# minaskar/pocomc

Hardware: AMD Instinct MI355X
Metric: preconditioned MCMC steps/sec (1e4 particles, 32-D) (higher is better)
Workload: dtype f32 flow (MFMA) + f64 step

## Files before the change

include/pocomc_amd.h:

```cpp
#ifndef POCOMC_AMD_H
#define POCOMC_AMD_H

#include <stdint.h>

#ifdef __cplusplus
extern "C" {
#endif

#define PMC_ABI_VERSION 9

const char* pmc_last_error(void);
int pmc_abi_version(void);
const char* pmc_build_id(void);


typedef struct pmc_maf {
    const float* packed;
    const int32_t* meta;
    int32_t D, H, T;
    int32_t Hp, Dp;
    int32_t nT, nXT, nOT;
    int64_t pk_per_transform;
    int32_t tri_ok;
    int32_t n_out;
    const uint16_t* lane16;
    int32_t lane16_fmt;
    int32_t reserved;
} pmc_maf_t;

#define PMC_MAF_VARIANT_LEFT_LOOKING 1
#define PMC_MAF_VARIANT_LANE_FOUR 2

#define PMC_INVERSE_AUTO 0
#define PMC_INVERSE_TRIANGULAR 1
#define PMC_INVERSE_NAIVE 2
#define PMC_INVERSE_TRIANGULAR_SOLO 6
#define PMC_INVERSE_TRIANGULAR_LANE 8
#define PMC_INVERSE_TRIANGULAR_LANE16 9
#define PMC_INVERSE_TRIANGULAR_DUO 7

int pmc_maf_pack(const float* flat, const int32_t* pack_idx, float* packed, int64_t n_packed, void* stream);

int pmc_maf_forward(const pmc_maf_t* m, const float* x, float* z, float* ladj, float* log_prob,
                    int64_t n, void* stream);

int pmc_maf_pack_bf16(const float* flat, const int32_t* pack_idx, uint16_t* image, int64_t n, void* stream);
// ... 280 lines not shown

#define PMC_ADAPT_TPCN 1
#define PMC_ADAPT_PRWM 2
#define PMC_ADAPT_RWM 3
#define PMC_ADAPT_MU 8

int pmc_rng_fill(const pmc_rng_t* rng, double gamma_shape, double* normal, double* gamma, double* uniform,
                 int64_t n, int32_t D, void* stream);
int pmc_event_synchronize(void* ev);

int pmc_propose_inverse(int kind, const float* cur32, const double* mu, const double* inv_cov, const double* chol,
                        double nu, double sigma, double cn_a, const pmc_rng_t* rng, double* prop64, double* quad,
                        double* quad_prop, const pmc_maf_t* maf, float* u_out, float* ladj, int64_t n, void* stream);

int pmc_step_pre(const pmc_step_t* s, const pmc_rng_t* rng, double nu, double sigma, double cn_a, void* stream);
int pmc_step_post(const pmc_step_t* s, const pmc_rng_t* rng, double beta, double nu, int want_mask,
                  int copy_sums, void* stream);
int pmc_step_lik_rows(const pmc_step_t* s, void* stream);
int pmc_step_prior_rows(const pmc_step_t* s, const void* logp, int logp_is_f32, void* stream);
int pmc_adapt_update(const double* const* parts, int32_t n_parts, int32_t D, double* total_out, double* h_sums,
                     double* adapt_state, int32_t adapt_mode, double c_sigma, double c_mu, double cap, double n_total,
                     const pmc_done_t* done, void* stream);
int pmc_stream_synchronize(void* stream);

void* pmc_comm_create(int32_t rank, int32_t world, int32_t width);
void* pmc_comm_create_host(int32_t rank, int32_t world, int32_t width);
int pmc_comm_kind(void* comm);
int pmc_comm_unlink(void* comm);
int pmc_comm_handle(void* comm, void* out64);
int pmc_comm_connect(void* comm, const void* handles);
// ... 82 lines not shown
```

pocomc_amd/_lib.py:

```python
from __future__ import annotations

import ctypes as C
import os

_HERE = os.path.dirname(os.path.abspath(__file__))
LIB_PATH = os.environ.get("PMC_LIBRARY") or os.path.join(_HERE, "libpocomc_amd.so")

c_p = C.c_void_p


class pmc_maf_t(C.Structure):
    _fields_ = [("packed", c_p), ("meta", c_p),
                ("D", C.c_int32), ("H", C.c_int32), ("T", C.c_int32),
                ("Hp", C.c_int32), ("Dp", C.c_int32),
                ("nT", C.c_int32), ("nXT", C.c_int32), ("nOT", C.c_int32),
                ("pk_per_transform", C.c_int64),
                ("tri_ok", C.c_int32), ("n_out", C.c_int32),
                ("lane16", c_p), ("lane16_fmt", C.c_int32), ("reserved", C.c_int32)]


class pmc_maf_train_t(C.Structure):
    _fields_ = [("packedT", c_p), ("gmap", c_p), ("pkT_per_transform", C.c_int64),
                ("gmap_per_transform", C.c_int64),
                ("jobs", c_p), ("n_jobs", C.c_int32), ("max_sets", C.c_int32), ("n_sq_partial", C.c_int32),
# ... 110 lines not shown
    "pmc_scaler_forward": (C.c_int, [P(pmc_scaler_t), c_p, c_p, i64, c_p]),
    "pmc_prior_logpdf": (C.c_int, [P(pmc_prior_t), c_p, c_p, c_p, i64, c_p]),
    "pmc_scaler_inverse_prior": (C.c_int, [P(pmc_scaler_t), P(pmc_prior_t), c_p, c_p, c_p, c_p, c_p, c_p, c_p, c_p,
                                           c_p, c_p, P(pmc_done_t), i64, c_p]),
    "pmc_wait_flag": (C.c_int, [c_p, i64, f64]),
    "pmc_propose": (C.c_int, [C.c_int, c_p, c_p, c_p, c_p, c_p, f64, f64, f64, P(pmc_rng_t),
                              c_p, c_p, c_p, c_p, i64, i32, c_p]),
    "pmc_accept_workspace_bytes": (i64, [i64, i32]),
    "pmc_accept": (C.c_int, [C.c_int, C.c_int, P(pmc_state_t), P(pmc_proposal_t), f64, f64,
                             P(pmc_rng_t), c_p, c_p, c_p, c_p, i64, i32, c_p]),
    "pmc_accept_armed": (C.c_int, [C.c_int, C.c_int, P(pmc_state_t), P(pmc_proposal_t), f64, f64,
                                   P(pmc_rng_t), c_p, c_p, c_p, c_p, P(pmc_done_t), c_p, i64, i32, c_p]),
    "pmc_propose_inverse": (C.c_int, [C.c_int, c_p, c_p, c_p, c_p, f64, f64, f64, P(pmc_rng_t), c_p, c_p, c_p,
                                      P(pmc_maf_t), c_p, c_p, i64, c_p]),
    "pmc_step_pre": (C.c_int, [P(pmc_step_t), P(pmc_rng_t), f64, f64, f64, c_p]),
    "pmc_step_post": (C.c_int, [P(pmc_step_t), P(pmc_rng_t), f64, f64, C.c_int, C.c_int, c_p]),
    "pmc_step_lik_rows": (C.c_int, [P(pmc_step_t), c_p]),
    "pmc_step_prior_rows": (C.c_int, [P(pmc_step_t), c_p, C.c_int, c_p]),
    "pmc_stream_synchronize": (C.c_int, [c_p]),
    "pmc_pipeline_create": (C.c_void_p, [C.POINTER(C.c_void_p), i32, C.c_uint64, C.POINTER(C.c_uint64), c_p, f64, c_p]),
    "pmc_pipeline_set_comm": (C.c_int, [c_p, c_p]),
    "pmc_comm_create": (C.c_void_p, [i32, i32, i32]),
    "pmc_comm_create_host": (C.c_void_p, [i32, i32, i32]),
    "pmc_comm_kind": (C.c_int, [c_p]),
    "pmc_comm_unlink": (C.c_int, [c_p]),
    "pmc_comm_handle": (C.c_int, [c_p, c_p]),
    "pmc_comm_connect": (C.c_int, [c_p, c_p]),
    "pmc_comm_destroy": (None, [c_p]),
    "pmc_comm_adapt_update": (C.c_int, [c_p, C.POINTER(C.c_void_p), i32, i32, c_p, c_p, c_p, i32, f64, f64, f64, f64, P(pmc_done_t), f64,
                                        c_p]),
# ... 120 lines not shown
```

pocomc_amd/csrc/maf_inverse_tri4.hip:

```cpp

#include <stdlib.h>
#include "maf_chain_rot.h"

#define DG_WORDS(m) ((m)->nT * 4 + 8)
#define TRI5_TT_WORDS(m) (((m)->nT + 2) * 16)
#define TRI5_YT_WORDS(m) ((m)->T * (((m)->nT + 2) * 4 + 1))
#define TRI5_TABLE_WORDS(m) (((TRI5_TT_WORDS(m) + (m)->Dp + 2 * (m)->T + 3) & ~3) + (m)->Dp * 16 + ((TRI5_YT_WORDS(m) + 3) & ~3))
#define TRI5_LDS_FLOATS(m, maxo) (2 * (m)->Dp * 16 + 2 * (m)->Hp * 16 + 2 * 256 + 2 * (3 + (maxo)) * 256 + TRI5_TABLE_WORDS(m))
#include "propose_body.h"

#define PX4 2
#define PK4 8


template <int TT>
__device__ __forceinline__ void burst_tile_open(f32x4& a1, f32x4& a2, f32x4& c1, f32x4& c2, const float4 (&pf1)[PK4],
                                                const float4 (&pf2)[PK4], const float* H0, const float* H1, int lane) {
    if constexpr (TT > 0) {
        float4 b1[TT], b2[TT];
#pragma unroll
        for (int i = 0; i < TT; ++i) {
            b1[i] = *reinterpret_cast<const float4*>(H0 + (i << 8) + (lane << 2));
            b2[i] = *reinterpret_cast<const float4*>(H1 + (i << 8) + (lane << 2));
        }
// ... 514 lines not shown
        else if constexpr (K == 11) F.w0o[3] = make_float4(0.f, 0.f, 0.f, 0.f);
        else F.w0N[K - 12] = bload4(rs, U + 1 < nT ? ((K - 12) << 6) + vo_q : OOB_VOFF, base + oCW0 + Un * 1024);
    };
    auto take_table = [&](ChainFrags<MAXO>& F, const int tt, const int U) {
        const int4 ty = *reinterpret_cast<const int4*>(YT + (tt * (nT + 2) + U) * 4);
        F.yo[0] = ty.x; F.yo[1] = ty.y; F.yo[2] = ty.z; F.yo[3] = ty.w;
        const int4 tg = *reinterpret_cast<const int4*>(DGT + 16 * U);
        const int4 txy = *reinterpret_cast<const int4*>(DGT + 16 * U + 4);
        const int4 tso = *reinterpret_cast<const int4*>(DGT + 16 * U + 8);
        F.g[0] = tg.x & 0xffff; F.g[1] = tg.y; F.g[2] = tg.z; F.g[3] = tg.w;
        F.pat = tg.x >> 16;
        F.xy[0] = txy.x; F.xy[1] = txy.y; F.xy[2] = txy.z; F.xy[3] = txy.w;
        F.so[0] = tso.x; F.so[1] = tso.y; F.so[2] = tso.z; F.so[3] = tso.w;
    };

    ChainFrags<MAXO> fA, fB;
    if (wv < TRI5_NC) {
        fill_table();
        WAVE_LDS_FENCE();
        {
            auto woff = [](const int r) { return 4 * (((r >> 4) << 8) + ((r & 3) << 6) + ((r >> 2) & 3)); };
            auto src_rank = [&](const int tt, const int g) {
                if (g >= D) return 0;
                return tt == T - 1 ? g : rank_of_feat[(tt + 1) * D + feat_of_rank[tt * D + g]];
            };
            for (int e = lane; e < T * (nT + 2) * 4; e += 64) {
                const int tt = e / ((nT + 2) * 4), rem = e - tt * (nT + 2) * 4;
                YT[e] = woff(src_rank(tt, DGT[16 * (rem >> 2) + (rem & 3)] & 0xffff));
            }
            for (int tt = lane; tt < T; tt += 64) Y0T[tt] = woff(src_rank(tt, 0));
        }
        WAVE_LDS_FENCE();
        {
            const int4 w0 = *reinterpret_cast<const int4*>(DGT + 12), w1 = *reinterpret_cast<const int4*>(DGT + 16 + 12);
            take_table(fA, T - 1, 0);
            static_for<16>([&](auto k_) { request(fA, k_, T - 1, 0, w0, w1); });
        }
        if constexpr (FM > 0) {
            for (int e = lane; e < (Dp - D) * 16; e += 64) Y[lidx(D + (e >> 4), e & 15)] = 0.0f;
            const double sg = pa.adapt ? pa.adapt[0] : pa.sigma, ca = pa.adapt ? pa.adapt[1] : pa.cn_a;
            propose_body<FM>(pa.kind, pa.cur32, nullptr, pa.adapt ? pa.adapt + 2 : pa.mu, pa.inv_cov, pa.chol, pa.nu, sg,
                             ca, pa.rng, pa.prop64, nullptr, pa.quad, pa.quad_prop, n, D, Y, rank_of_feat + (T - 1) * D,
                             set);
        } else {
            load_rows(Y, in, row0, n, D, Dp, feat_of_rank + (T - 1) * D, lane);
        }
    } else {
        float4* z4 = reinterpret_cast<float4*>(H0);
        const int n4 = (2 * Hp * 16 + 2 * 256 + 2 * TRI5_STAGE_FLOATS(MAXO)) >> 2;
        for (int e = lane; e < n4; e += 64) z4[e] = make_float4(0.f, 0.f, 0.f, 0.f);
    }
    if (pa.prof && lane == 0 && blockIdx.x < 64)
        pa.prof[(size_t)T * nT * 8 + blockIdx.x * 2 + wv] = (long long)__builtin_amdgcn_s_getreg((31 << 11) | 4);
    for (int r = threadIdx.x; r < D; r += 64 * (TRI5_NC + 1)) PRM[r] = feat_of_rank[r];
    for (int tt = threadIdx.x; tt < T; tt += 64 * (TRI5_NC + 1)) {
        const float* b3 = m.packed + (size_t)tt * m.pk_per_transform + (oB3 >> 2);
        B3T[2 * tt] = b3[0];
        B3T[2 * tt + 1] = b3[1];
    }
    for (int e = threadIdx.x; e < (Dp * 16) >> 2; e += 64 * (TRI5_NC + 1)) {
        reinterpret_cast<float4*>(XA)[e] = make_float4(0.f, 0.f, 0.f, 0.f);
        reinterpret_cast<float4*>(XB)[e] = make_float4(0.f, 0.f, 0.f, 0.f);
    }
    float ladj = 0.0f;
    int xsel = 0;
    __syncthreads();

#define BURST_FETCH(TB, TT, P1, P2, XF, OF, Bz0, Bz1, Bz2)                                                        \
            {    \
                 \
                const int TT_ = (TT) < nT ? (TT) : nT - 1;                                                        \
                const int so1_ = (TB) + oF1 + TT_ * nT * 1024, so2_ = (TB) + oF2 + TT_ * nT * 1024;               \
                _Pragma("unroll") for (int i_ = 0; i_ < PK4; ++i_) {                                              \
// ... 305 lines not shown
```

pocomc_amd/csrc/scaler_body.h:

```cpp
#ifndef PMC_SCALER_BODY_H
#define PMC_SCALER_BODY_H

#include <hip/hip_runtime.h>
#include <math.h>
#include <stdint.h>
#include "../../include/pocomc_amd.h"

#pragma clang fp contract(off)

#define LOG_SQRT_2PI 0.91893853320467267
#define SQRT2 1.4142135623730951

__device__ __forceinline__ double np_pairwise_leaf(const double* a, int n) {
    if (n < 8) {
        double res = 0.0;
        for (int i = 0; i < n; ++i) res += a[i];
        return res;
    }
    double r0 = a[0], r1 = a[1], r2 = a[2], r3 = a[3], r4 = a[4], r5 = a[5], r6 = a[6], r7 = a[7];
    int i;
    for (i = 8; i < n - (n % 8); i += 8) {
        r0 += a[i + 0]; r1 += a[i + 1]; r2 += a[i + 2]; r3 += a[i + 3];
        r4 += a[i + 4]; r5 += a[i + 5]; r6 += a[i + 6]; r7 += a[i + 7];
    }
// ... 124 lines not shown
    }
    e.u_out[g] = u;
    e.x_out[g] = x;
    if (direct_cm) { if (e.x_colmajor) e.x_colmajor[(size_t)j * n + row0 + r] = x; }
    else Xt[j * 17 + r] = x;
    Jt[r * D + j] = J;
    if (e.have_prior) Pt[r * D + j] = prior_term(e.pr, j, x);
    if (!isfinite(x)) rowfin[r] = 0;
}

__device__ __forceinline__ void scaler_epilogue_rows(const ScalerEpi& e, const double* Jt, const double* Pt, const double* Xt,
                                                     int* rowfin, int64_t row0, int64_t n, int D, int tid, int nthr,
                                                     bool cm_done) {
    const pmc_scaler_t& s = e.s;
    const int rows = (int)min((int64_t)16, n - row0);
    if (tid < rows) {
        double l = np_pairwise_sum(Jt + (size_t)tid * D, D);
        if (s.scale) l = s.sum_log_sigma + l;
        e.ldj_out[row0 + tid] = l;
        const int fin = (rowfin[tid] && isfinite(l)) ? 1 : 0;
        e.finite_out[row0 + tid] = fin;
        if (e.finite_copy) e.finite_copy[row0 + tid] = fin;
        bool clean = fin != 0;
        if (e.have_prior) {
            double lp = -INFINITY;
            if (fin) {
                lp = 0.0;
                for (int j = 0; j < D; ++j) lp += Pt[tid * D + j];
            }
            e.logp_out[row0 + tid] = lp;
            if (e.logp_copy) e.logp_copy[row0 + tid] = lp;
            clean = clean && isfinite(lp);
        }
        if (e.bad_count && !clean) atomicAdd(e.bad_count, 1u);
        if (e.fill_x) rowfin[tid] = clean ? 1 : 0;
    }
    if (e.fill_x) __syncthreads();
    if (e.stamps && tid == 0) e.stamps[blockIdx.x * 8 + 2] = wall_clock64();
    if (e.stamps && tid == 0) e.stamps[blockIdx.x * 8 + 3] = wall_clock64();
    if (e.x_colmajor && !cm_done) {
        for (int el = tid; el < rows * D; el += nthr) {
            const int j = el / rows, r = el - j * rows;
            e.x_colmajor[(size_t)j * n + row0 + r] = (e.fill_x && !rowfin[r]) ? e.fill_x[(row0 + r) * D + j] : Xt[j * 17 + r];
        }
    }
    if (e.stamps && tid == 0) e.stamps[blockIdx.x * 8 + 4] = wall_clock64();
    if (e.done_flag) {
        __builtin_amdgcn_fence(__ATOMIC_RELEASE, "agent");
        __syncthreads();
        if (e.stamps && tid == 0) e.stamps[blockIdx.x * 8 + 5] = wall_clock64();
        if (tid == 0) {
            const unsigned t = __hip_atomic_fetch_add(e.done_ticket, 1u, __ATOMIC_ACQ_REL, __HIP_MEMORY_SCOPE_AGENT);
            if (t == gridDim.x - 1) {
                *e.done_ticket = 0u;
                if (e.bad_count && e.bad_flag) {
                    const unsigned bad = __hip_atomic_exchange(e.bad_count, 0u, __ATOMIC_ACQ_REL, __HIP_MEMORY_SCOPE_AGENT);
                    *e.bad_flag = (long long)bad;
                }
// ... 4 lines not shown
    }
}

template <class LIDX>
__device__ __forceinline__ void scaler_epilogue(const ScalerEpi& e, const float* X, const int* __restrict__ rof,
                                                double* scr, int64_t row0, int64_t n, int D, int tid, int nthr,
                                                LIDX lidx_of) {
    double* Jt = scr;
    double* Pt = Jt + 16 * D;
    double* Xt = Pt + 16 * D;
    int* rowfin = reinterpret_cast<int*>(Xt + D * 17);
    const int rows = (int)min((int64_t)16, n - row0);
    if (tid < 16) rowfin[tid] = 1;
    if (e.stamps && tid == 0) e.stamps[blockIdx.x * 8 + 0] = wall_clock64();
    __syncthreads();
    for (int el = tid; el < rows * D; el += nthr) {
        const int r = el / D, j = el - r * D;
        scaler_epilogue_element(e, Jt, Pt, Xt, rowfin, X[lidx_of(rof[j], r)], r, j, row0, n, D, false);
    }
    __syncthreads();
    if (e.stamps && tid == 0) e.stamps[blockIdx.x * 8 + 1] = wall_clock64();
    scaler_epilogue_rows(e, Jt, Pt, Xt, rowfin, row0, n, D, tid, nthr, false);
}

static inline size_t scaler_progressive_lds_bytes(int D) { return (size_t)(2 * 16 * D) * sizeof(double) + 16 * sizeof(int); }

#endif
```

pocomc_amd/csrc/step.hip:

```cpp

#include <hip/hip_runtime.h>
#include <time.h>
#include "pmc_internal.h"
#include "scaler_body.h"

#ifdef PMC_DEBUG_HOOKS
static long long* g_epilogue_stamps = nullptr;
static int64_t g_epilogue_stamps_n = 0;
#endif

extern "C" int pmc_step_pre(const pmc_step_t* s, const pmc_rng_t* rng, double nu, double sigma, double cn_a,
                            void* stream) {
    if (!s || !rng) return pmc_fail("pmc_step_pre: null argument");
    hipStream_t st = (hipStream_t)stream;
    const int64_t n = s->n;
    const int32_t D = s->D;
    const bool tpcn = (s->kind == PMC_KIND_TPCN);
    pmc_rng_t rr = *rng;
    const bool prefill = s->rng_ready && s->rng_normal[0] && s->rng_normal[1] && s->rng_uniform[0] &&
                         s->rng_uniform[1] && (!tpcn || (s->rng_gamma[0] && s->rng_gamma[1])) && !rng->normal &&
                         !rng->gamma && !rng->uniform;
    const int rb = (int)(rng->step & 1);
    const double gshape = tpcn ? 0.5 * ((double)D + nu) : 0.0;
    if (prefill) {
        if (*s->rng_ready != (int64_t)rng->step) {
            int rcf = pmc_rng_fill(rng, gshape, s->rng_normal[rb], s->rng_gamma[rb], s->rng_uniform[rb], n, D, stream);
            if (rcf) return rcf;
        }
        rr.normal = s->rng_normal[rb];
        rr.gamma = tpcn ? s->rng_gamma[rb] : nullptr;
        rng = &rr;
    }
    auto finish = [&]() -> int {
        if (s->ev_pre_done) (void)hipEventRecord((hipEvent_t)s->ev_pre_done, st);
        if (prefill) {
            pmc_rng_t nx = *rng;
            nx.normal = nullptr; nx.gamma = nullptr; nx.uniform = nullptr;
            nx.step = rng->step + 1;
            int rcf = pmc_rng_fill(&nx, gshape, s->rng_normal[rb ^ 1], s->rng_gamma[rb ^ 1], s->rng_uniform[rb ^ 1], n, D,
                                   stream);
            if (rcf) return rcf;
            *s->rng_ready = (int64_t)nx.step;
        }
        return 0;
    };
    const bool direct = s->host_direct && !s->p_xT;
    const double* mu = s->mu;
    const double* adapt = (s->adapt_state && s->adapt_mode) ? s->adapt_state : nullptr;
    if (!adapt && tpcn && s->h_mu) {
        if (direct) mu = s->h_mu;
        else if (hipMemcpyAsync((void*)s->mu, s->h_mu, (size_t)D * sizeof(double), hipMemcpyHostToDevice, st) != hipSuccess)
            return pmc_fail("pmc_step_pre: H2D mu");
    }
    int rc;
    bool fused = false;
    int scaled = 0;
    const pmc_prior_t* pr = s->prior;
    double* lp = pr ? s->p_logp : nullptr;
// ... 64 lines not shown
                                         lp, fin2, lp2, done, n, stream, &sx);
    }
    if (rc) return rc;
    if (direct || devlik) return finish();
    if (pr) {
        if (hipMemcpyAsync(s->h_logp_out, s->p_logp, (size_t)n * sizeof(double), hipMemcpyDeviceToHost, st) != hipSuccess)
            return pmc_fail("pmc_step_pre: D2H logp");
    }
    const double* xsrc = s->p_xT ? s->p_xT : s->p_x;
    if (hipMemcpyAsync(s->h_x, xsrc, (size_t)n * D * sizeof(double), hipMemcpyDeviceToHost, st) != hipSuccess ||
        hipMemcpyAsync(s->h_fin, s->p_fin, (size_t)n * sizeof(int32_t), hipMemcpyDeviceToHost, st) != hipSuccess)
        return pmc_fail("pmc_step_pre: D2H");
    return finish();
}

__global__ __launch_bounds__(256) void lik_rows_kernel(const double* __restrict__ x_prop, const double* __restrict__ x_cur,
                                                       const int32_t* __restrict__ fin, const double* __restrict__ logp,
                                                       double* __restrict__ lik_x, unsigned* __restrict__ bad_count,
                                                       int64_t n, int D) {
    const int64_t r = (int64_t)blockIdx.x * 256 + threadIdx.x;
    if (r >= n) return;
    const bool reach = fin[r] && isfinite(logp[r]);
    const double* src = (reach ? x_prop : x_cur) + r * D;
    for (int j = 0; j < D; ++j) lik_x[(size_t)j * n + r] = src[j];
    if (!reach) atomicAdd(bad_count, 1u);
}

extern "C" int pmc_step_lik_rows(const pmc_step_t* s, void* stream) {
    if (!s || !s->lik_x || !s->clean_count || !s->p_x || !s->cur.x || !s->p_fin || !s->p_logp || !s->h_logp || s->D < 1)
        return pmc_fail("pmc_step_lik_rows: needs lik_x, clean_count, p_x, cur.x, p_fin, p_logp and h_logp");
// ... 219 lines not shown

extern "C" void pmc_pipeline_destroy(void* pp) { delete (pmc_pipeline*)pp; }

extern "C" int pmc_pipeline_set_comm(void* pp, void* comm) {
    pmc_pipeline* p = (pmc_pipeline*)pp;
    if (!p) return pmc_fail("pmc_pipeline_set_comm: null pipeline");
    p->comm = comm;
    return 0;
}

static int pipeline_enqueue_pre(pmc_pipeline* p, int64_t step, double nu) {
    for (int k = 0; k < p->n_lanes; ++k) {
        pmc_step_t s = *p->lanes[k];
        s.adapt_mode = 1;
        p->rng[k].step = (uint64_t)step;
        const int rc = pmc_step_pre(&s, &p->rng[k], nu, 0.0, 0.0, p->stream);
        if (rc) return rc;
        if (p->prefetcher)
            (void)pmc_prefetcher_submit(p->prefetcher, s.h_done, step + 1, s.h_x, (int64_t)s.n * s.D * 8, p->timeout > 0 ? p->timeout : 1.0);
    }
    return 0;
}

extern "C" int pmc_pipeline_start(void* pp, double nu, int64_t first_step) {
    pmc_pipeline* p = (pmc_pipeline*)pp;
    if (!p) return pmc_fail("pmc_pipeline_start: null pipeline");
    p->step = first_step;
    return pipeline_enqueue_pre(p, first_step, nu);
}

extern "C" int pmc_pipeline_next(void* pp, int32_t lane_done, double beta, double nu, int32_t adapt_mode, double c_sigma,
                                 double c_mu, double cap, double n_total, int32_t more) {
    pmc_pipeline* p = (pmc_pipeline*)pp;
    if (!p || lane_done < -1 || lane_done >= p->n_lanes) return pmc_fail("pmc_pipeline_next: bad argument");
// ... 56 lines not shown
```

pocomc_amd/flow.py:

```python
from __future__ import annotations

import ctypes as C
import warnings

import numpy as np
import torch

from . import _lib
from .maf_spec import MAFSpec, SPEC_BY_NAME, NSF_BY_NAME, spec_by_name


def torch_double_to_float(x: torch.Tensor, warn: bool = True) -> torch.Tensor:
    if x.dtype == torch.float64 and warn:
        warnings.warn("Float64 data is currently unsupported, casting to Float32. "
                      "Output will also have type Float32.")
        return x.float()
    elif x.dtype == torch.float32:
        return x
    raise ValueError(f"Unsupported datatype for input data: {x.dtype}")


LANE16_BOUND = 1e-2
LANE16_LADJ_BOUND = 1e-1
LANE16_LADJ_Q99_BOUND = 5e-2
# ... 16 lines not shown
        self.spec = spec
        self.lib = _lib.load()
        self.device = torch.device(device) if device is not None else _lib.require_gpu()
        if self.device.type != "cuda":
            raise _lib.PocomcAmdError("Flow lives on the GPU; there is no CPU fallback")
        if seed is None:
            seed = int(torch.randint(0, 2 ** 31 - 1, (1,)).item())
        self.params = torch.from_numpy(spec.init_params(seed)).to(self.device)
        self._pack_idx = torch.from_numpy(spec.pack_index()).to(self.device)
        self._meta = torch.from_numpy(spec.device_meta()).to(self.device)
        self._packed = torch.zeros(spec.pk_size, dtype=torch.float32, device=self.device)
        self._desc = _lib.pmc_maf_t(
            packed=self._packed.data_ptr(), meta=self._meta.data_ptr(),
            D=spec.n_dim, H=spec.hidden, T=spec.n_transforms, Hp=spec.Hp, Dp=spec.Dp,
            nT=spec.nT, nXT=spec.nXT, nOT=spec.nOT, pk_per_transform=spec.pk_per_transform,
            tri_ok=int(spec.tri_ok), n_out=spec.n_out)
        self.inverse_algo = 0
        if precision not in ("f32", "bf16"):
            raise ValueError("precision must be 'f32' or 'bf16'")
        if precision == "bf16" and spec.univariate != "affine":
            raise NotImplementedError("the bf16 kernels are built for the affine flows")
        self.precision = precision
        if train_engine not in (None, "f32", "bf16"):
            raise ValueError("train_engine must be None, 'f32' or 'bf16'")
        self.train_engine = train_engine
        if inverse_precision is None:
            inverse_precision = "f32"
        if inverse_precision not in ("f32", "bf16", "f16"):
            raise ValueError("inverse_precision must be 'f32', 'bf16' or 'f16'")
        if inverse_precision != "f32" and spec.univariate != "affine":
            raise NotImplementedError("the 16-bit helper products are built for the affine flows")
# ... 188 lines not shown
```

pocomc_amd/maf_spec.py:

```python
from __future__ import annotations

import math
from dataclasses import dataclass, field

import numpy as np

LOG_SLOPE = math.log(1e-3)


def next_power_of_2(n: int) -> int:
    return 1 if n == 0 else 2 ** (int(n) - 1).bit_length()


def default_hidden(n_dim: int) -> int:
    return max(next_power_of_2(3 * n_dim), 32)


def _ceil_to(x: int, m: int) -> int:
    return (x + m - 1) // m * m


@dataclass
class MAFSpec:

# ... 275 lines not shown
                    b3i[r, :NO] = base_c + off3 + NO * feat + np.arange(NO)
                put("f3i", f3i); put("b3i", b3i)
        return idx.astype(np.int32)

    def tile_groups(self):
        out = []
        for T in range(self.nT):
            dq = self.quad_deg[4 * T:4 * T + 4]
            g = []
            for d in dq:
                if d < self.n_dim and (not g or g[-1] != d):
                    g.append(int(d))
            out.append(g)
        return out

    def device_meta(self) -> np.ndarray:
        D, T = self.n_dim, self.n_transforms
        live = int(np.sum((self.quad_deg.reshape(-1, 4) < D).any(axis=1)))
        hdr = np.array([D, self.hidden, T, self.Hp, self.Dp, self.nT,
                        self.pk_per_transform, live], dtype=np.int32)
        f_o_r = np.concatenate([np.argsort(o) for o in self.orders]).astype(np.int32)
        r_o_f = np.concatenate(self.orders).astype(np.int32)
        return np.concatenate([hdr, f_o_r, r_o_f, self.quad_meta]).astype(np.int32)

    def bf16_layout(self):
        nX2, nK2 = -(-self.Dp // 32), -(-self.Hp // 32)
        sz = {"g0": self.nT * nX2 * 512, "g1": self.nT * nK2 * 512, "g2": self.nT * nK2 * 512, "g3": self.nOT * nK2 * 512}
        off, o = {}, 0
        for k, v in sz.items():
            off[k] = o
            o += v
        return dict(nX2=nX2, nK2=nK2, sz=sz, off=off, per_transform=o)

    def pack_index_bf16(self) -> np.ndarray:
        D, H = self.n_dim, self.hidden
        L = self.bf16_layout()
        nX2, nK2, nT, nOT = L["nX2"], L["nK2"], self.nT, self.nOT
        idx = np.full(L["per_transform"] * self.n_transforms, -1, dtype=np.int64)
# ... 294 lines not shown
```

pocomc_amd/mcmc.py:

```python
from __future__ import annotations

import ctypes as C
import os
import time
from functools import partial

import numpy as np
import torch
import torch.distributed as dist

from . import _lib

KINDS = ("preconditioned_pcn", "preconditioned_rwm", "pcn", "rwm")
PMC_KIND_TPCN, PMC_KIND_RWM = 0, 1


def _env_wait_timeout(): return float(os.environ.get("PMC_WAIT_TIMEOUT", "600"))
def _env_no_fuse(): return int(os.environ.get("PMC_NO_FUSE", "0"))
def _env_c_pipeline(): return os.environ.get("PMC_C_PIPELINE", "1") != "0"
def _env_c_allreduce(): return os.environ.get("PMC_C_ALLREDUCE", "1") != "0"
def _env_comm_mailbox(): return os.environ.get("PMC_COMM_MAILBOX", "")


PMC_ADAPT_TPCN, PMC_ADAPT_PRWM, PMC_ADAPT_RWM, PMC_ADAPT_MU = 1, 2, 3, 8
# ... 497 lines not shown
                              offset=self.offset)

    def can_pipeline(self):
        return bool(not self._instrumented() and self.host_direct and self.x_order == "F"
                    and self.spin_wait and self.D <= 256)

    def adapt_upload(self, sigma, mu=None):
        a = self._h_adapt.numpy()
        a[0] = sigma
        a[1] = (1.0 - sigma ** 2.0) ** 0.5 if self.tpcn else 0.0
        a[2:] = 0.0 if mu is None else mu
        self.adapt_state.copy_(self._h_adapt, non_blocking=True)
        self._step.adapt_state = self.adapt_state.data_ptr()
        self.device_adapt = True

    def propose(self, sigma, nu=0.0, replay=None, step=None):
        if self._instrumented():
            return self._propose_instrumented(sigma, nu, replay)
        if replay is not None:
            self._rng_cur = self._rng(replay)
        else:
            self._rng_fast.step = self.step_idx if step is None else int(step)
            self._rng_cur = self._rng_fast
        self._step.adapt_mode = 1 if self.device_adapt else 0
        self._configure_step()
        if self.device_adapt:
            sigma, cn_a = 0.0, 0.0
        else:
            cn_a = float((1.0 - sigma ** 2.0) ** 0.5) if self.tpcn else 0.0
        self._stream = self.stream.cuda_stream if self.stream is not None else _lib.stream_handle()
        _lib.check(self.lib.pmc_step_pre(C.byref(self._step), C.byref(self._rng_cur), float(nu), float(sigma), cn_a,
                                         self._stream), "pmc_step_pre")
        if self.prefetcher is not None and self._direct_now:
            self.lib.pmc_prefetcher_submit(self.prefetcher, self.h_done.data_ptr(), int(self._rng_cur.step) + 1,
                                           self.h_x.data_ptr(), self.n * self.D * 8, self.wait_timeout)

    def _propose_instrumented(self, sigma, nu, replay):
        lib, n, D = self.lib, self.n, self.D
        self._np_clean[0] = -1
        self._rng_cur = self._rng(replay)
        st = _lib.stream_handle()
        kind = PMC_KIND_TPCN if self.tpcn else PMC_KIND_RWM
        cn_a = float((1.0 - sigma ** 2.0) ** 0.5) if self.tpcn else 0.0
        with torch.cuda.device(self.device):
            e0 = self._ev()
            _lib.check(lib.pmc_propose(
                kind, _lib.ptr(self.theta32) if self.pre else None, None if self.pre else _lib.ptr(self.u),
                _lib.ptr(self.mu_d), _lib.ptr(self.inv_cov_d), _lib.ptr(self.chol_d), float(nu), float(sigma), cn_a,
                C.byref(self._rng_cur), _lib.ptr(self.p_theta64), _lib.ptr(self.p_theta32) if self.pre else None,
                _lib.ptr(self.quad) if self.tpcn else None, _lib.ptr(self.p_quad) if self.tpcn else None,
# ... 320 lines not shown
            for e in self.lanes:
                e._configure_step()
            assert all(e._direct_now for e in self.lanes)
            self._lane_structs = (C.c_void_p * K)(*[C.addressof(e._step) for e in self.lanes])
            offs = (C.c_uint64 * K)(*[e.offset for e in self.lanes])
            stream = first.stream.cuda_stream if first.stream is not None else _lib.stream_handle()
            first._stream = stream
            self._pipe = self.lib.pmc_pipeline_create(self._lane_structs, K, first.seed, offs, first.prefetcher,
                                                      float(first.wait_timeout), stream)
            if not self._pipe:
                _lib.check(1, "pmc_pipeline_create")
            if comm:
                _lib.check(self.lib.pmc_pipeline_set_comm(self._pipe, comm), "pmc_pipeline_set_comm")
            _lib.check(self.lib.pmc_pipeline_start(self._pipe, float(nu), int(first.step_idx)), "pmc_pipeline_start")
            return
        for e in self.lanes:
            e.host_timers = self.host_timers
            e.propose(None, nu)

    def resume_pipeline(self, nu):
        first = self.lanes[0]
        if self._pipe:
            _lib.check(self.lib.pmc_pipeline_start(self._pipe, float(nu), int(first.step_idx)), "pmc_pipeline_start")
            return
        for e in self.lanes:
            e.host_timers = self.host_timers
            e.propose(None, nu, step=e.step_idx)

    def pipeline_stats(self, reset=True):
        if not self._pipe:
            return None
        out = (C.c_double * 6)()
        _lib.check(self.lib.pmc_pipeline_stats(self._pipe, out, int(reset)), "pmc_pipeline_stats")
        return dict(wait_x=out[0], wait_sums=out[1], enqueue_accept=out[2], enqueue_next_pre=out[3], steps=int(out[4]))

    def step_pipelined(self, beta, nu, coefficients, n_total, log_prior, log_like, more=True):
        if self._pipe:
            nxt, P = self.lib.pmc_pipeline_next, self._pipe
            mode, c_sigma, c_mu, cap = coefficients
            tm = self.host_timers
            if nxt(P, -1, beta, nu, mode, c_sigma, c_mu, cap, n_total, 0):
                _lib.check(1, "pmc_pipeline_next")
# ... 29 lines not shown
                e.accept_enqueue(beta, nu, host_sums=False)
            if tm is not None:
                tm["enqueue_accept"] = tm.get("enqueue_accept", 0.0) + clock() - t0
        t0 = clock() if tm is not None else 0.0
        stream = self.lanes[0]._stream
        if sharded:
            mode, c_sigma, c_mu, cap = coefficients
            self._flag_value += 1
            done = _lib.pmc_done_t(flag=self._h_flag.data_ptr(), value=self._flag_value, ticket=None)
            state = self.lanes[0].adapt_state.data_ptr()
            allreduce_sums(self._tot, self.group)
            _lib.check(lib.pmc_adapt_update(self._tot_part, 1, D, None, self._h_tot.data_ptr(), state, mode, c_sigma,
                                            c_mu, cap, float(n_total), C.byref(done), stream), "pmc_adapt_update")
        t1 = clock() if tm is not None else 0.0
        if more:
            for e in self.lanes:
                e.propose(None, nu, step=e.step_idx + 1)
        t2 = clock() if tm is not None else 0.0
        if sharded:
            _lib.check(lib.pmc_wait_flag(self._h_flag.data_ptr(), self._flag_value, self.lanes[0].wait_timeout), "pmc_wait_flag")
            sums = self._h_tot.numpy()
        else:
            sums = last.accept_wait()
        if tm is not None:
            t3 = clock()
            tm["enqueue_adapt"] = tm.get("enqueue_adapt", 0.0) + t1 - t0
            tm["enqueue_next_pre"] = tm.get("enqueue_next_pre", 0.0) + t2 - t1
            tm["wait_sums"] = tm.get("wait_sums", 0.0) + t3 - t2
        for e in (self.lanes if sharded else self.lanes[:-1]):
            e.step_idx += 1
        return calls, sums

# ... 325 lines not shown
```

Before: 3324.

## Precompute sweep tables, defer RNG prefill, and parallelize scaler epilogue reductions

Result: faster. 3430, median of 6 (+3.2%).

```diff
diff --git a/include/pocomc_amd.h b/include/pocomc_amd.h
--- a/include/pocomc_amd.h
+++ b/include/pocomc_amd.h
@@ -30,6 +30,7 @@
 
 #define PMC_MAF_VARIANT_LEFT_LOOKING 1
 #define PMC_MAF_VARIANT_LANE_FOUR 2
+#define PMC_MAF_TABLES 4
 
 #define PMC_INVERSE_AUTO 0
 #define PMC_INVERSE_TRIANGULAR 1
@@ -340,6 +341,8 @@
                         double* quad_prop, const pmc_maf_t* maf, float* u_out, float* ladj, int64_t n, void* stream);
 
 int pmc_step_pre(const pmc_step_t* s, const pmc_rng_t* rng, double nu, double sigma, double cn_a, void* stream);
+int pmc_step_pre_deferred(const pmc_step_t* s, const pmc_rng_t* rng, double nu, double sigma, double cn_a, void* stream);
+int pmc_step_fill_next(const pmc_step_t* s, const pmc_rng_t* rng, double nu, void* stream);
 int pmc_step_post(const pmc_step_t* s, const pmc_rng_t* rng, double beta, double nu, int want_mask,
                   int copy_sums, void* stream);
 int pmc_step_lik_rows(const pmc_step_t* s, void* stream);
diff --git a/pocomc_amd/_lib.py b/pocomc_amd/_lib.py
--- a/pocomc_amd/_lib.py
+++ b/pocomc_amd/_lib.py
@@ -148,6 +148,8 @@
     "pmc_propose_inverse": (C.c_int, [C.c_int, c_p, c_p, c_p, c_p, f64, f64, f64, P(pmc_rng_t), c_p, c_p, c_p,
                                       P(pmc_maf_t), c_p, c_p, i64, c_p]),
     "pmc_step_pre": (C.c_int, [P(pmc_step_t), P(pmc_rng_t), f64, f64, f64, c_p]),
+    "pmc_step_pre_deferred": (C.c_int, [P(pmc_step_t), P(pmc_rng_t), f64, f64, f64, c_p]),
+    "pmc_step_fill_next": (C.c_int, [P(pmc_step_t), P(pmc_rng_t), f64, c_p]),
     "pmc_step_post": (C.c_int, [P(pmc_step_t), P(pmc_rng_t), f64, f64, C.c_int, C.c_int, c_p]),
     "pmc_step_lik_rows": (C.c_int, [P(pmc_step_t), c_p]),
     "pmc_step_prior_rows": (C.c_int, [P(pmc_step_t), c_p, C.c_int, c_p]),
diff --git a/pocomc_amd/csrc/maf_inverse_tri4.hip b/pocomc_amd/csrc/maf_inverse_tri4.hip
--- a/pocomc_amd/csrc/maf_inverse_tri4.hip
+++ b/pocomc_amd/csrc/maf_inverse_tri4.hip
@@ -552,8 +552,21 @@
         F.so[0] = tso.x; F.so[1] = tso.y; F.so[2] = tso.z; F.so[3] = tso.w;
     };
 
+    const bool tabs = (m.reserved & PMC_MAF_TABLES) != 0;
+    const int* tabg = m.meta + ((8 + 2 * T * D + 4 * nT + 3) & ~3);
+    const int tab_words = TRI5_TT_WORDS(&m) + Dp;
     ChainFrags<MAXO> fA, fB;
-    if (wv < TRI5_NC) {
+    if (wv < TRI5_NC && tabs) {
+        const int4* tg4 = reinterpret_cast<const int4*>(tabg);
+        const int4 ty = *reinterpret_cast<const int4*>(tabg + tab_words + ((T - 1) * (nT + 2)) * 4);
+        const int4 tg = tg4[0], txy = tg4[1], tso = tg4[2], w0 = tg4[3], w1 = tg4[4 + 3];
+        fA.yo[0] = ty.x; fA.yo[1] = ty.y; fA.yo[2] = ty.z; fA.yo[3] = ty.w;
+        fA.g[0] = tg.x & 0xffff; fA.g[1] = tg.y; fA.g[2] = tg.z; fA.g[3] = tg.w;
+        fA.pat = tg.x >> 16;
+        fA.xy[0] = txy.x; fA.xy[1] = txy.y; fA.xy[2] = txy.z; fA.xy[3] = txy.w;
+        fA.so[0] = tso.x; fA.so[1] = tso.y; fA.so[2] = tso.z; fA.so[3] = tso.w;
+        static_for<16>([&](auto k_) { request(fA, k_, T - 1, 0, w0, w1); });
+    } else if (wv < TRI5_NC) {
         fill_table();
         WAVE_LDS_FENCE();
         {
@@ -574,6 +587,8 @@
             take_table(fA, T - 1, 0);
             static_for<16>([&](auto k_) { request(fA, k_, T - 1, 0, w0, w1); });
         }
+    }
+    if (wv < TRI5_NC) {
         if constexpr (FM > 0) {
             for (int e = lane; e < (Dp - D) * 16; e += 64) Y[lidx(D + (e >> 4), e & 15)] = 0.0f;
             const double sg = pa.adapt ? pa.adapt[0] : pa.sigma, ca = pa.adapt ? pa.adapt[1] : pa.cn_a;
@@ -587,14 +602,27 @@
         float4* z4 = reinterpret_cast<float4*>(H0);
         const int n4 = (2 * Hp * 16 + 2 * 256 + 2 * TRI5_STAGE_FLOATS(MAXO)) >> 2;
         for (int e = lane; e < n4; e += 64) z4[e] = make_float4(0.f, 0.f, 0.f, 0.f);
+        if (tabs) {
+            const int4* src = reinterpret_cast<const int4*>(tabg);
+            for (int e = lane; e < tab_words >> 2; e += 64) reinterpret_cast<int4*>(DGT)[e] = src[e];
+            src = reinterpret_cast<const int4*>(tabg + tab_words);
+            for (int e = lane; e < (TRI5_YT_WORDS(&m) + 3) >> 2; e += 64) reinterpret_cast<int4*>(YT)[e] = src[e];
+            for (int tt = lane; tt < T; tt += 64) {
+                const float* b3 = m.packed + (size_t)tt * m.pk_per_transform + (oB3 >> 2);
+                B3T[2 * tt] = b3[0];
+                B3T[2 * tt + 1] = b3[1];
+            }
+        }
     }
     if (pa.prof && lane == 0 && blockIdx.x < 64)
         pa.prof[(size_t)T * nT * 8 + blockIdx.x * 2 + wv] = (long long)__builtin_amdgcn_s_getreg((31 << 11) | 4);
-    for (int r = threadIdx.x; r < D; r += 64 * (TRI5_NC + 1)) PRM[r] = feat_of_rank[r];
-    for (int tt = threadIdx.x; tt < T; tt += 64 * (TRI5_NC + 1)) {
-        const float* b3 = m.packed + (size_t)tt * m.pk_per_transform + (oB3 >> 2);
-        B3T[2 * tt] = b3[0];
-        B3T[2 * tt + 1] = b3[1];
+    if (!tabs) {
+        for (int r = threadIdx.x; r < D; r += 64 * (TRI5_NC + 1)) PRM[r] = feat_of_rank[r];
+        for (int tt = threadIdx.x; tt < T; tt += 64 * (TRI5_NC + 1)) {
+            const float* b3 = m.packed + (size_t)tt * m.pk_per_transform + (oB3 >> 2);
+            B3T[2 * tt] = b3[0];
+            B3T[2 * tt + 1] = b3[1];
+        }
     }
     for (int e = threadIdx.x; e < (Dp * 16) >> 2; e += 64 * (TRI5_NC + 1)) {
         reinterpret_cast<float4*>(XA)[e] = make_float4(0.f, 0.f, 0.f, 0.f);
diff --git a/pocomc_amd/csrc/scaler_body.h b/pocomc_amd/csrc/scaler_body.h
--- a/pocomc_amd/csrc/scaler_body.h
+++ b/pocomc_amd/csrc/scaler_body.h
@@ -162,34 +162,66 @@
                                                      bool cm_done) {
     const pmc_scaler_t& s = e.s;
     const int rows = (int)min((int64_t)16, n - row0);
-    if (tid < rows) {
-        double l = np_pairwise_sum(Jt + (size_t)tid * D, D);
-        if (s.scale) l = s.sum_log_sigma + l;
-        e.ldj_out[row0 + tid] = l;
-        const int fin = (rowfin[tid] && isfinite(l)) ? 1 : 0;
-        e.finite_out[row0 + tid] = fin;
-        if (e.finite_copy) e.finite_copy[row0 + tid] = fin;
-        bool clean = fin != 0;
-        if (e.have_prior) {
-            double lp = -INFINITY;
-            if (fin) {
-                lp = 0.0;
-                for (int j = 0; j < D; ++j) lp += Pt[tid * D + j];
-            }
-            e.logp_out[row0 + tid] = lp;
-            if (e.logp_copy) e.logp_copy[row0 + tid] = lp;
-            clean = clean && isfinite(lp);
-        }
-        if (e.bad_count && !clean) atomicAdd(e.bad_count, 1u);
-        if (e.fill_x) rowfin[tid] = clean ? 1 : 0;
+    const int n8 = D - (D % 8);
+    for (int rb = 0; rb < 16; rb += nthr >> 3) {
+        const int r = rb + (tid >> 3), i = tid & 7;
+        const bool live = r < rows;
+        const double* a = Jt + (size_t)r * D;
+        double acc = 0.0;
+        if (live && D >= 8) {
+            acc = a[i];
+            for (int k = i + 8; k < n8; k += 8) acc += a[k];
+        }
+        double lps = 0.0;
+        if (live && e.have_prior && i == 4) {
+            const double* P = Pt + (size_t)r * D;
+            int j = 0;
+            for (; j + 8 <= D; j += 8) {
+                const double p0 = P[j], p1 = P[j + 1], p2 = P[j + 2], p3 = P[j + 3];
+                const double p4 = P[j + 4], p5 = P[j + 5], p6 = P[j + 6], p7 = P[j + 7];
+                lps += p0; lps += p1; lps += p2; lps += p3; lps += p4; lps += p5; lps += p6; lps += p7;
+            }
+            for (; j < D; ++j) lps += P[j];
+        }
+        acc = acc + __shfl_xor(acc, 1, 8);
+        acc = acc + __shfl_xor(acc, 2, 8);
+        acc = acc + __shfl_xor(acc, 4, 8);
+        lps = __shfl(lps, 4, 8);
+        if (live && i == 0) {
+            double l;
+            if (D < 8) {
+                l = 0.0;
+                for (int k = 0; k < D; ++k) l += a[k];
+            } else {
+                l = acc;
+                for (int k = n8; k < D; ++k) l += a[k];
+            }
+            if (s.scale) l = s.sum_log_sigma + l;
+            e.ldj_out[row0 + r] = l;
+            const int fin = (rowfin[r] && isfinite(l)) ? 1 : 0;
+            e.finite_out[row0 + r] = fin;
+            if (e.finite_copy) e.finite_copy[row0 + r] = fin;
+            bool clean = fin != 0;
+            if (e.have_prior) {
+                const double lp = fin ? lps : -INFINITY;
+                e.logp_out[row0 + r] = lp;
+                if (e.logp_copy) e.logp_copy[row0 + r] = lp;
+                clean = clean && isfinite(lp);
+            }
+            if (e.bad_count && !clean) atomicAdd(e.bad_count, 1u);
+            if (e.fill_x) rowfin[r] = clean ? 1 : 0;
+        }
     }
     if (e.fill_x) __syncthreads();
     if (e.stamps && tid == 0) e.stamps[blockIdx.x * 8 + 2] = wall_clock64();
     if (e.stamps && tid == 0) e.stamps[blockIdx.x * 8 + 3] = wall_clock64();
     if (e.x_colmajor && !cm_done) {
+        const int dj = nthr / rows, dr = nthr - dj * rows;
+        int j = tid / rows, r = tid - j * rows;
         for (int el = tid; el < rows * D; el += nthr) {
-            const int j = el / rows, r = el - j * rows;
             e.x_colmajor[(size_t)j * n + row0 + r] = (e.fill_x && !rowfin[r]) ? e.fill_x[(row0 + r) * D + j] : Xt[j * 17 + r];
+            j += dj; r += dr;
+            if (r >= rows) { r -= rows; ++j; }
         }
     }
     if (e.stamps && tid == 0) e.stamps[blockIdx.x * 8 + 4] = wall_clock64();
@@ -224,9 +256,14 @@
     if (tid < 16) rowfin[tid] = 1;
     if (e.stamps && tid == 0) e.stamps[blockIdx.x * 8 + 0] = wall_clock64();
     __syncthreads();
-    for (int el = tid; el < rows * D; el += nthr) {
-        const int r = el / D, j = el - r * D;
-        scaler_epilogue_element(e, Jt, Pt, Xt, rowfin, X[lidx_of(rof[j], r)], r, j, row0, n, D, false);
+    {
+        const int dr = nthr / D, dj = nthr - dr * D;
+        int r = tid / D, j = tid - r * D;
+        for (int el = tid; el < rows * D; el += nthr) {
+            scaler_epilogue_element(e, Jt, Pt, Xt, rowfin, X[lidx_of(rof[j], r)], r, j, row0, n, D, false);
+            r += dr; j += dj;
+            if (j >= D) { j -= D; ++r; }
+        }
     }
     __syncthreads();
     if (e.stamps && tid == 0) e.stamps[blockIdx.x * 8 + 1] = wall_clock64();
diff --git a/pocomc_amd/csrc/step.hip b/pocomc_amd/csrc/step.hip
--- a/pocomc_amd/csrc/step.hip
+++ b/pocomc_amd/csrc/step.hip
@@ -9,17 +9,34 @@
 static int64_t g_epilogue_stamps_n = 0;
 #endif
 
-extern "C" int pmc_step_pre(const pmc_step_t* s, const pmc_rng_t* rng, double nu, double sigma, double cn_a,
-                            void* stream) {
+static bool step_prefills(const pmc_step_t* s, const pmc_rng_t* rng) {
+    return s->rng_ready && s->rng_normal[0] && s->rng_normal[1] && s->rng_uniform[0] && s->rng_uniform[1] &&
+           (s->kind != PMC_KIND_TPCN || (s->rng_gamma[0] && s->rng_gamma[1])) && !rng->normal && !rng->gamma && !rng->uniform;
+}
+
+extern "C" int pmc_step_fill_next(const pmc_step_t* s, const pmc_rng_t* rng, double nu, void* stream) {
+    if (!s || !rng) return pmc_fail("pmc_step_fill_next: null argument");
+    if (!step_prefills(s, rng)) return 0;
+    const int rb = (int)(rng->step & 1);
+    const double gshape = (s->kind == PMC_KIND_TPCN) ? 0.5 * ((double)s->D + nu) : 0.0;
+    pmc_rng_t nx = *rng;
+    nx.step = rng->step + 1;
+    int rcf = pmc_rng_fill(&nx, gshape, s->rng_normal[rb ^ 1], s->rng_gamma[rb ^ 1], s->rng_uniform[rb ^ 1], s->n, s->D, stream);
+    if (rcf) return rcf;
+    *s->rng_ready = (int64_t)nx.step;
+    return 0;
+}
+
+static int step_pre(const pmc_step_t* s, const pmc_rng_t* rng, double nu, double sigma, double cn_a, void* stream,
+                    bool fill_next) {
     if (!s || !rng) return pmc_fail("pmc_step_pre: null argument");
     hipStream_t st = (hipStream_t)stream;
     const int64_t n = s->n;
     const int32_t D = s->D;
     const bool tpcn = (s->kind == PMC_KIND_TPCN);
     pmc_rng_t rr = *rng;
-    const bool prefill = s->rng_ready && s->rng_normal[0] && s->rng_normal[1] && s->rng_uniform[0] &&
-                         s->rng_uniform[1] && (!tpcn || (s->rng_gamma[0] && s->rng_gamma[1])) && !rng->normal &&
-                         !rng->gamma && !rng->uniform;
+    const bool prefill = step_prefills(s, rng);
+    const pmc_rng_t* rng_in = rng;
     const int rb = (int)(rng->step & 1);
     const double gshape = tpcn ? 0.5 * ((double)D + nu) : 0.0;
     if (prefill) {
@@ -33,15 +50,7 @@
     }
     auto finish = [&]() -> int {
         if (s->ev_pre_done) (void)hipEventRecord((hipEvent_t)s->ev_pre_done, st);
-        if (prefill) {
-            pmc_rng_t nx = *rng;
-            nx.normal = nullptr; nx.gamma = nullptr; nx.uniform = nullptr;
-            nx.step = rng->step + 1;
-            int rcf = pmc_rng_fill(&nx, gshape, s->rng_normal[rb ^ 1], s->rng_gamma[rb ^ 1], s->rng_uniform[rb ^ 1], n, D,
-                                   stream);
-            if (rcf) return rcf;
-            *s->rng_ready = (int64_t)nx.step;
-        }
+        if (prefill && fill_next) return pmc_step_fill_next(s, rng_in, nu, stream);
         return 0;
     };
     const bool direct = s->host_direct && !s->p_xT;
@@ -136,6 +145,16 @@
     return finish();
 }
 
+extern "C" int pmc_step_pre(const pmc_step_t* s, const pmc_rng_t* rng, double nu, double sigma, double cn_a,
+                            void* stream) {
+    return step_pre(s, rng, nu, sigma, cn_a, stream, true);
+}
+
+extern "C" int pmc_step_pre_deferred(const pmc_step_t* s, const pmc_rng_t* rng, double nu, double sigma, double cn_a,
+                                     void* stream) {
+    return step_pre(s, rng, nu, sigma, cn_a, stream, false);
+}
+
 __global__ __launch_bounds__(256) void lik_rows_kernel(const double* __restrict__ x_prop, const double* __restrict__ x_cur,
                                                        const int32_t* __restrict__ fin, const double* __restrict__ logp,
                                                        double* __restrict__ lik_x, unsigned* __restrict__ bad_count,
@@ -385,10 +404,14 @@
         pmc_step_t s = *p->lanes[k];
         s.adapt_mode = 1;
         p->rng[k].step = (uint64_t)step;
-        const int rc = pmc_step_pre(&s, &p->rng[k], nu, 0.0, 0.0, p->stream);
+        const int rc = step_pre(&s, &p->rng[k], nu, 0.0, 0.0, p->stream, false);
         if (rc) return rc;
         if (p->prefetcher)
             (void)pmc_prefetcher_submit(p->prefetcher, s.h_done, step + 1, s.h_x, (int64_t)s.n * s.D * 8, p->timeout > 0 ? p->timeout : 1.0);
+    }
+    for (int k = 0; k < p->n_lanes; ++k) {
+        const int rc = pmc_step_fill_next(p->lanes[k], &p->rng[k], nu, p->stream);
+        if (rc) return rc;
     }
     return 0;
 }
diff --git a/pocomc_amd/flow.py b/pocomc_amd/flow.py
--- a/pocomc_amd/flow.py
+++ b/pocomc_amd/flow.py
@@ -8,6 +8,8 @@
 
 from . import _lib
 from .maf_spec import MAFSpec, SPEC_BY_NAME, NSF_BY_NAME, spec_by_name
+
+PMC_MAF_TABLES = 4
 
 
 def torch_double_to_float(x: torch.Tensor, warn: bool = True) -> torch.Tensor:
@@ -54,7 +56,8 @@
             packed=self._packed.data_ptr(), meta=self._meta.data_ptr(),
             D=spec.n_dim, H=spec.hidden, T=spec.n_transforms, Hp=spec.Hp, Dp=spec.Dp,
             nT=spec.nT, nXT=spec.nXT, nOT=spec.nOT, pk_per_transform=spec.pk_per_transform,
-            tri_ok=int(spec.tri_ok), n_out=spec.n_out)
+            tri_ok=int(spec.tri_ok), n_out=spec.n_out,
+            reserved=PMC_MAF_TABLES if spec.has_sweep_tables else 0)
         self.inverse_algo = 0
         if precision not in ("f32", "bf16"):
             raise ValueError("precision must be 'f32' or 'bf16'")
diff --git a/pocomc_amd/maf_spec.py b/pocomc_amd/maf_spec.py
--- a/pocomc_amd/maf_spec.py
+++ b/pocomc_amd/maf_spec.py
@@ -313,6 +313,59 @@
             out.append(g)
         return out
 
+    @property
+    def has_sweep_tables(self) -> bool:
+        return bool(self.n_out == 2 and self.tri_ok and self.nOT <= 8 and self.n_dim <= 64)
+
+    def sweep_tables(self) -> np.ndarray:
+        D, T, nT, Dp = self.n_dim, self.n_transforms, self.nT, self.Dp
+        oob = 0x40000000
+        f_o_r = [np.argsort(o) for o in self.orders]
+        r_o_f = self.orders
+        deg = (self.quad_meta & 0xffff).astype(np.int64)
+        dgt = np.zeros((nT + 2, 16), dtype=np.int64)
+        for tile in range(nT + 2):
+            g4, pat = [D] * 4, 1
+            if tile < nT:
+                x, y, z, w = (int(v) for v in deg[4 * tile:4 * tile + 4])
+                ny, nz, nw = y != x, z != y, w != z
+                pat = 1 | (ny << 1) | (nz << 2) | (nw << 3)
+                g1 = y if ny else (z if nz else (w if nw else D))
+                g2 = (z if nz else (w if nw else D)) if ny else (w if (nz and nw) else D)
+                g3 = w if (ny and nz and nw) else D
+                g4 = [x, g1, g2, g3]
+            for k in range(16):
+                i = k & 3
+                g = g4[i]
+                live = g < D
+                gg = g if live else 0
+                if k < 4:
+                    v = g | ((pat << 16) if i == 0 else 0)
+                elif k < 8:
+                    v = 4 * (((gg >> 4) << 8) + ((gg & 3) << 6) + ((gg >> 2) & 3))
+                elif k < 12:
+                    v = 4 * ((gg >> 3) * 256 + 2 * (gg & 7))
+                else:
+                    v = (((((gg >> 3) * nT) << 6) + 2 * (gg & 7)) << 4) if live else oob
+                dgt[tile, k] = v
+        woff = lambda r: 4 * (((r >> 4) << 8) + ((r & 3) << 6) + ((r >> 2) & 3))
+
+        def src_rank(tt, g):
+            if g >= D:
+                return 0
+            return g if tt == T - 1 else int(r_o_f[tt + 1][f_o_r[tt][g]])
+        yt = np.zeros((T, nT + 2, 4), dtype=np.int64)
+        for tt in range(T):
+            for tile in range(nT + 2):
+                for i in range(4):
+                    yt[tt, tile, i] = woff(src_rank(tt, int(dgt[tile, i]) & 0xffff))
+        y0t = np.array([woff(src_rank(tt, 0)) for tt in range(T)], dtype=np.int64)
+        prm = np.zeros(Dp, dtype=np.int64)
+        prm[:D] = f_o_r[0]
+        tail = np.concatenate([yt.reshape(-1), y0t])
+        tail = np.concatenate([tail, np.zeros(-len(tail) % 4, dtype=np.int64)])
+        return np.concatenate([dgt.reshape(-1), prm, tail]).astype(np.int32)
+
     def device_meta(self) -> np.ndarray:
         D, T = self.n_dim, self.n_transforms
         live = int(np.sum((self.quad_deg.reshape(-1, 4) < D).any(axis=1)))
@@ -320,7 +373,10 @@
                         self.pk_per_transform, live], dtype=np.int32)
         f_o_r = np.concatenate([np.argsort(o) for o in self.orders]).astype(np.int32)
         r_o_f = np.concatenate(self.orders).astype(np.int32)
-        return np.concatenate([hdr, f_o_r, r_o_f, self.quad_meta]).astype(np.int32)
+        meta = np.concatenate([hdr, f_o_r, r_o_f, self.quad_meta]).astype(np.int32)
+        if self.has_sweep_tables:
+            meta = np.concatenate([meta, np.zeros(-len(meta) % 4, dtype=np.int32), self.sweep_tables()])
+        return meta
 
     def bf16_layout(self):
         nX2, nK2 = -(-self.Dp // 32), -(-self.Hp // 32)
diff --git a/pocomc_amd/mcmc.py b/pocomc_amd/mcmc.py
--- a/pocomc_amd/mcmc.py
+++ b/pocomc_amd/mcmc.py
@@ -535,7 +535,7 @@
         self._step.adapt_state = self.adapt_state.data_ptr()
         self.device_adapt = True
 
-    def propose(self, sigma, nu=0.0, replay=None, step=None):
+    def propose(self, sigma, nu=0.0, replay=None, step=None, defer_fill=False):
         if self._instrumented():
             return self._propose_instrumented(sigma, nu, replay)
         if replay is not None:
@@ -550,11 +550,17 @@
         else:
             cn_a = float((1.0 - sigma ** 2.0) ** 0.5) if self.tpcn else 0.0
         self._stream = self.stream.cuda_stream if self.stream is not None else _lib.stream_handle()
-        _lib.check(self.lib.pmc_step_pre(C.byref(self._step), C.byref(self._rng_cur), float(nu), float(sigma), cn_a,
-                                         self._stream), "pmc_step_pre")
+        pre = self.lib.pmc_step_pre_deferred if defer_fill else self.lib.pmc_step_pre
+        _lib.check(pre(C.byref(self._step), C.byref(self._rng_cur), float(nu), float(sigma), cn_a, self._stream), "pmc_step_pre")
         if self.prefetcher is not None and self._direct_now:
             self.lib.pmc_prefetcher_submit(self.prefetcher, self.h_done.data_ptr(), int(self._rng_cur.step) + 1,
                                            self.h_x.data_ptr(), self.n * self.D * 8, self.wait_timeout)
+
+    def fill_next(self, nu=0.0):
+        if self._instrumented():
+            return
+        _lib.check(self.lib.pmc_step_fill_next(C.byref(self._step), C.byref(self._rng_cur), float(nu), self._stream),
+                   "pmc_step_fill_next")
 
     def _propose_instrumented(self, sigma, nu, replay):
         lib, n, D = self.lib, self.n, self.D
@@ -905,18 +911,21 @@
                 _lib.check(self.lib.pmc_pipeline_set_comm(self._pipe, comm), "pmc_pipeline_set_comm")
             _lib.check(self.lib.pmc_pipeline_start(self._pipe, float(nu), int(first.step_idx)), "pmc_pipeline_start")
             return
+        self._propose_lanes(nu)
+
+    def _propose_lanes(self, nu, ahead=0):
         for e in self.lanes:
             e.host_timers = self.host_timers
-            e.propose(None, nu)
+            e.propose(None, nu, step=e.step_idx + ahead, defer_fill=True)
+        for e in self.lanes:
+            e.fill_next(nu)
 
     def resume_pipeline(self, nu):
         first = self.lanes[0]
         if self._pipe:
             _lib.check(self.lib.pmc_pipeline_start(self._pipe, float(nu), int(first.step_idx)), "pmc_pipeline_start")
             return
-        for e in self.lanes:
-            e.host_timers = self.host_timers
-            e.propose(None, nu, step=e.step_idx)
+        self._propose_lanes(nu)
 
     def pipeline_stats(self, reset=True):
         if not self._pipe:
@@ -976,8 +985,7 @@
                                             c_mu, cap, float(n_total), C.byref(done), stream), "pmc_adapt_update")
         t1 = clock() if tm is not None else 0.0
         if more:
-            for e in self.lanes:
-                e.propose(None, nu, step=e.step_idx + 1)
+            self._propose_lanes(nu, ahead=1)
         t2 = clock() if tm is not None else 0.0
         if sharded:
             _lib.check(lib.pmc_wait_flag(self._h_flag.data_ptr(), self._flag_value, self.lanes[0].wait_timeout), "pmc_wait_flag")
```
